# batra-mlp-lab/visdial

Measured on AMD Instinct MI355X. Metric: QA-rounds/sec training mn-att-ques-im-hist+disc (batch 20x10x100), higher is better.
Workload: dtype f32 operands and results; the option recurrence multiplies the EXACT 3-way bf16 split of both operands (9 bf16 MFMA products per fp32 product, f32 accumulate: fp32-grade, errors at the f32 MFMA's own level) -- its two step kernels and its weight-gradient contraction; f32 MFMA (v_mfma_f32_32x32x2_f32

## Files before the change

visdial_amd/csrc/common.h:

```cpp
#pragma once
#include <hip/hip_runtime.h>
#include <stdint.h>
#include <stdio.h>
#include <string.h>

#define VD_OK 0
#define VD_ERR_ARG -1
#define VD_ERR_HIP -2
#define VD_ERR_STATE -3
#define VD_FLAG_BF16 1
#define VD_FLAG_SPLIT9 2
#define VD_FLAG_SPLIT6 4
#define VD_FLAG_SPLIT3 8
#define VD_FLAG_SPLIT (VD_FLAG_SPLIT9 | VD_FLAG_SPLIT6 | VD_FLAG_SPLIT3)
#define VD_FLAG_LIVE_PREFIX 16
#define VD_FLAG_STATE_ONLY 32
#define VD_FLAG_TREE 64
#define VD_FLAG_HOLD 128
#define VD_LIVE_PREFIX_ROWS 128
#define VD_BEAM_LMAX 64

void vd_set_error(const char* fmt, ...);

#define VD_CHECK_ARG(cond, ...)                                   \
// ... 32 lines not shown
  float* wht = nullptr;
  size_t wht_bytes = 0;
  unsigned* sync = nullptr;
  size_t sync_bytes = 0;
};
int vd_stream_scratch(hipStream_t stream, size_t wht_bytes, size_t sync_bytes, VdStreamScratch* out);
int vd_num_cus();

struct VdZeroSet {
  float* buf[6];
  int ncols[6];
  int n;
  long quads_per_row;
};
int vd_zero_inactive_multi(const VdZeroSet& z, const int32_t* nact_dev, int T, int N, hipStream_t stream);

typedef unsigned short vd_bf16_bits;
int vd_lstm_forward_c16(const vd_bf16_bits* table16, int64_t tab_ld, const int32_t* tok_gather, const float* Wh, vd_bf16_bits* gates16,
                        vd_bf16_bits* h16, float* h_last, float* c, int T, int N, int H, hipStream_t stream);
int vd_lstm_backward_c16(const float* Wh, vd_bf16_bits* gates16, const float* c, const float* dh_last, float* dc_work, int T, int N, int H,
                         hipStream_t stream);
int vd_f32_to_bf16(const float* src, vd_bf16_bits* dst, int64_t n, hipStream_t stream);
int vd_gemm_tn_acc_bf16(const vd_bf16_bits* A16, const vd_bf16_bits* B16, float* C, int64_t ldc, int M, int N, int K, hipStream_t stream);
int vd_segment_rowsum_acc_bf16(const vd_bf16_bits* X16, int64_t ldx, const int32_t* tok, const int32_t* perm, int64_t n, int ncol,
                               float* out, int64_t ldo, hipStream_t stream);

int vd_bf16_shadow_get(int slot, const float* base, size_t floats, vd_bf16_bits** out);
const vd_bf16_bits* vd_bf16_shadow_find(const float* p, size_t floats);
void vd_bf16_shadow_invalidate(const float* p, size_t floats);

// ... 70 lines not shown
```

visdial_amd/csrc/gemm_core.h:

```cpp
#pragma once
#include <stdint.h>
#include <stdlib.h>
#include <type_traits>

#include "common.h"

#ifdef VD_TIMING
#define VD_TSLOTS 12
#define VD_TBLOCKS 8192
static __device__ unsigned long long vd_tbuf[VD_TBLOCKS * VD_TSLOTS];
#define VD_TSTAMP(i, clk)                                                                \
  do {                                                                                   \
    if (threadIdx.x == 0 && blockIdx.x < VD_TBLOCKS) vd_tbuf[blockIdx.x * VD_TSLOTS + (i)] = (clk); \
  } while (0)
#define VD_T(i) VD_TSTAMP(i, __builtin_amdgcn_s_memtime())
#define VD_TREAL(i) VD_TSTAMP(i, __builtin_amdgcn_s_memrealtime())
#else
#define VD_T(i) do {} while (0)
#define VD_TREAL(i) do {} while (0)
#endif

template <int WM_, int WK_, int NT_, int KW_, int DB_ = 1, int MINW_ = 1, int LDSMIN_ = 0, int BF16_ = 0>
struct GemmCfg {
  static constexpr int WM = WM_, WK = WK_, NT = NT_, KW = KW_, DB = DB_, MINW = MINW_;
// ... 713 lines not shown
    attr_set = true;
  }
  const int rotate = rotate_in >= 0 ? rotate_in : 1;
  int grid = tiles_m * tiles_n * splits;
  if constexpr (EpiDeadOf<Epi>::value) {
    VD_CHECK_ARG(splits == 1, "launch_gemm_glds: an epilogue with a row-tile predicate takes no split-K");
    grid = (tiles_m + 7) / 8 * 8 * tiles_n;
  }
  const int lds = Cfg::LDS_BYTES;
  hipLaunchKernelGGL(kern, dim3(grid), dim3(Cfg::THREADS), lds, stream, M, N, K,
                     kchunk, tiles_m, tiles_n, rotate, A, lda, B, ldb, e);
  VD_LAUNCH_CHECK();
  return VD_OK;
}

template <class Prob, int MAXP>
struct GroupArgs {
  Prob p[MAXP];
  int tile_start[MAXP + 1];
  int nprob;
};

template <class Cfg, class Prob, int MAXP>
__global__ void __launch_bounds__(Cfg::THREADS, Cfg::MINW)
gemm_f32_grouped_kernel(GroupArgs<Prob, MAXP> g) {
  extern __shared__ __attribute__((aligned(16))) float smem[];
  if constexpr (Cfg::WK > 1) __builtin_amdgcn_s_setprio(3);
  const int wg = xcd_remap(blockIdx.x, gridDim.x);
  int pi = 0;
#pragma unroll
// ... 68 lines not shown
  __device__ __forceinline__ void operator()(const f32x16 (&acc)[NT], int row0, int col0, int lane, int M,
                                             int N, float*  = nullptr) const {
#pragma unroll
    for (int j = 0; j < NT; ++j) {
      const int col = col0 + j * 32 + (lane & 31);
      if (col >= N) continue;
#pragma unroll
      for (int r = 0; r < 16; ++r) {
        const int row = row0 + mfma_row(r, lane);
        if (row >= M) continue;
        unsafeAtomicAdd(C + (long)row * ldc + col, acc[j][r]);
      }
    }
  }
};

template <class Cfg, class ASrc, class BSrc, class Epi>
static int launch_gemm(int M, int N, int K, int splits, ASrc a, BSrc b, Epi e, hipStream_t stream) {
  if (M <= 0 || N <= 0) return VD_OK;
  const int tiles_m = vd_cdiv(M, Cfg::BM), tiles_n = vd_cdiv(N, Cfg::BN);
  if (splits < 1) splits = 1;
  int kchunk = K > 0 ? vd_cdiv(vd_cdiv(K, splits), Cfg::BK) * Cfg::BK : Cfg::BK;
  if (K > 0) splits = vd_cdiv(K, kchunk);
  else splits = 1;
  auto kern = gemm_f32_kernel<Cfg, ASrc, BSrc, Epi>;
  static bool attr_set = false;
  if (!attr_set) {
    VD_HIP(hipFuncSetAttribute(reinterpret_cast<const void*>(kern), hipFuncAttributeMaxDynamicSharedMemorySize,
                               Cfg::LDS_BYTES));
    attr_set = true;
// ... 13 lines not shown
```

visdial_amd/csrc/gemm_ops.hip:

```cpp
#include "gemm_core.h"
#include "split_core.h"

using CfgBigDB = GemmCfg<4, 1, 4, 32>;
using CfgBig = GemmCfg<4, 1, 4, 16, 0, 3>;
using CfgSmall = GemmCfg<1, 4, 1, 32, 0, 3>;

static inline bool use_small(int M, int N) {
  return (long)vd_cdiv(M, CfgBig::BM) * vd_cdiv(N, CfgBig::BN) < 48;
}

static int check_align(const void* p, long ld, const char* what) {
  if (((uintptr_t)p & 15) != 0 || (ld & 3) != 0) {
    vd_set_error("%s: pointer must be 16-byte aligned and leading dimension a multiple of 4 (ld=%ld)", what, ld);
    return VD_ERR_ARG;
  }
  return VD_OK;
}

__global__ void colsum_kernel(const float* __restrict__ X, long ld, int M, int N, int rows_per_block,
                              float* __restrict__ out) {
  const int col = blockIdx.x * blockDim.x + threadIdx.x;
  if (col >= N) return;
  const int r0 = blockIdx.y * rows_per_block;
  const int r1 = min(M, r0 + rows_per_block);
// ... 461 lines not shown
    return VD_OK;
  }
  const int cb = vd_cdiv(N, 256);
  int rb = vd_cdiv(1024, cb);
  int rows_per_block = vd_cdiv(M, rb);
  if (rows_per_block < 16) rows_per_block = 16;
  rb = vd_cdiv(M, rows_per_block);
  hipLaunchKernelGGL(colsum_kernel, dim3(cb, rb), dim3(256), 0, (hipStream_t)stream, X, ld, M, N,
                     rows_per_block, out);
  VD_LAUNCH_CHECK();
  return VD_OK;
}

}

__global__ void __launch_bounds__(256) bf16_tn_tail_kernel(const vd_bf16_bits* __restrict__ A, const vd_bf16_bits* __restrict__ B, float* __restrict__ C,
                                                           long ldc, int M, int N, int K) {
  const long i = (long)blockIdx.x * 256 + threadIdx.x;
  if (i >= (long)M * N) return;
  const int m = (int)(i / N), n = (int)(i % N);
  float acc = 0.f;
  for (int k = 0; k < K; ++k)
    acc += __uint_as_float((unsigned)A[(long)k * M + m] << 16) * __uint_as_float((unsigned)B[(long)k * N + n] << 16);
  unsafeAtomicAdd(C + (long)m * ldc + n, acc);
}
int vd_gemm_tn_acc_bf16(const vd_bf16_bits* A16, const vd_bf16_bits* B16, float* C, int64_t ldc, int M, int N, int K, hipStream_t stream) {
  VD_CHECK_ARG(A16 && B16 && C && M % 128 == 0 && N % 128 == 0 && K >= 0, "vd_gemm_tn_acc_bf16: M, N must be multiples of 128");
  const int K1 = K & ~31;
  if (K1 > 0) {
    const bool big = M % 256 == 0 && N % 256 == 0 && K1 >= 8192;
// ... 10 lines not shown
```

visdial_amd/csrc/paths.h:

```cpp
#pragma once
#include "common.h"

static inline int vd_precision_flags(int lstmBf16) {
  switch (lstmBf16) {
    case 0: return 0;
    case 1: return VD_FLAG_BF16;
    case 3: return VD_FLAG_SPLIT3;
    case 6: return VD_FLAG_SPLIT6;
    case 9: return VD_FLAG_SPLIT9;
    default: return -1;
  }
}
static inline int vd_split_nprod(int flags) {
  return (flags & VD_FLAG_SPLIT9) ? 9 : (flags & VD_FLAG_SPLIT6) ? 6 : (flags & VD_FLAG_SPLIT3) ? 3 : 0;
}

constexpr long VD_THROUGHPUT_ROWS = 2048;
constexpr int VD_LSTM_FWD_TILE_BIG = 128, VD_LSTM_FWD_TILE_SMALL = 32;
static inline int vd_lstm_fwd_row_tile(long N) { return N >= VD_THROUGHPUT_ROWS ? VD_LSTM_FWD_TILE_BIG : VD_LSTM_FWD_TILE_SMALL; }
static inline bool vd_lstm_glds_fwd_fits(long N, int H) { return N >= VD_THROUGHPUT_ROWS && H % 32 == 0 && N * H * 4 < (1L << 32); }
static inline bool vd_lstm_glds_bwd_fits(long N, int H) { return N >= VD_THROUGHPUT_ROWS && H % 32 == 0 && N * 4 * H * 4 < (1L << 32); }
static inline bool vd_lstm_bf16_fits(long N, int H) { return N >= VD_THROUGHPUT_ROWS && H % 32 == 0; }
static inline bool vd_lstm_c16_fits(long N, int H) { return N >= VD_THROUGHPUT_ROWS && H % 128 == 0; }

static inline bool vd_tn_kmajor_fits(long M, long N, long K) { return M % 128 == 0 && N % 128 == 0 && K >= 1024; }
constexpr int VD_SPLIT_TN_BM = 256, VD_SPLIT_TN_BN = 128;
static inline bool vd_tn_split_tiles(long M, long N) { return M % VD_SPLIT_TN_BM == 0 && N % VD_SPLIT_TN_BN == 0; }

static inline bool vd_img_split_ok(long rows, int H, int Kc) {
  return rows >= 128 && H % 16 == 0 && Kc % 16 == 0 && rows * (H > Kc ? H : Kc) * 4 < (1L << 32);
}

static inline bool vd_lhood_fused_fits(long rows, long ldh, long V, long ldw, int H) {
  return H >= 64 && H % 16 == 0 && V >= 128 && ldh % 4 == 0 && ldw % 4 == 0 && rows * ldh * 4 < (1L << 32) && V * ldw * 4 < (1L << 32);
}
static inline bool vd_lhood_prefix_fits(int T, long rows) { return T >= 1 && T < 256 && rows >= 1; }
```

visdial_amd/csrc/rt_core.h:

```cpp
#pragma once
#include <math.h>
#include <stdarg.h>
#include <stdlib.h>
#include <string.h>

#include <algorithm>
#include <map>
#include <memory>
#include <numeric>
#include <random>
#include <string>
#include <vector>

#include "../../include/visdial_hip.h"
#include "common.h"
#include "paths.h"
#include "rt_switches.h"

static_assert(VD_OK == 0 && VD_ERR_ARG == -1, "rt_switches.h returns the two as literals: it includes no common.h");

int vd_lstm2_forward_p(const vd_lstm2_fwd_t* st, int nstacks, int H, int flags, hipStream_t stream);
int vd_lstm2_backward_p(const vd_lstm2_bwd_t* st, int nstacks, int H, int flags, hipStream_t stream);

int vd_img_drop_gather(const float* pre, const uint8_t* mask1, float* xdrop, int N, int R, int S2, int H, float scale, hipStream_t stream);
int vd_img_common_forward_p(const float* pre, const uint8_t* mask1, const float* xdrop, const float* Wc, const float* bc, const float* qc,
                            const uint8_t* mask2, float* iqc, int N, int R, int S2, int H, int Kc, float scale, int flags, hipStream_t stream);
int vd_img_tr_backward_p(const float* dz, const float* Wc, const float* p, const float* datt, const uint8_t* mask1, float* dpre, int N, int R,
                         int S2, int H, int Kc, float scale, int flags, hipStream_t stream);
int vd_img_common_wgrad_p(const float* dz, const float* pre, const uint8_t* mask1, const float* xdrop, float* dWc, int N, int R, int S2, int H,
                          int Kc, float scale, int flags, hipStream_t stream);

int vd_mn_attention_round_p(const float* Q, int64_t q_ld, const float* Hm, float* P, float* hAtt, float* Qout, int B, int R, int r, int H,
// ... 59 lines not shown
};

struct DevBuf {
  void* p = nullptr;
  size_t bytes = 0;
};

struct SeqTok {
  int T = 0, N = 0;
  bool present = false, sorted = false;
  int32_t* tok = nullptr;
  std::vector<int32_t> nact;
  int32_t *tok_sorted = nullptr, *fwd_idx = nullptr, *inv_idx = nullptr, *perm = nullptr, *inv = nullptr, *nact_dev = nullptr;
  int32_t *act = nullptr, *act1 = nullptr, *prev1 = nullptr;
  int n_act = 0, n_act1 = 0;
};

struct TreeChunk {
  int o0 = 0, C = 0, Tl = 0, Nw = 0;
  long n_nodes = 0;
  std::vector<int32_t> widths;
  int32_t* mask2 = nullptr;
  int32_t* node_row = nullptr;
  int32_t *enode = nullptr, *etgt = nullptr;
};

struct BatchSlot {
  int B = 0;
  bool tree_ok = false;
  std::vector<TreeChunk> tree;
  SeqTok q, h, opt, ain, aout, oin, oout;
  float* img = nullptr;
  int32_t* gt = nullptr;
  std::vector<int32_t> gt_host;
  bool has_gt = false;
  int32_t* opt_uid = nullptr;
  int opt_total = 0;
  int32_t *opt_sort_off = nullptr, *opt_sort_perm = nullptr;
  bool cached = false;
  uint64_t cache_stamp = 0;
  std::vector<int32_t> miss_keys, opt_host;
  hipEvent_t ready = nullptr;
  hipEvent_t done = nullptr;
  bool used = false;
  bool uploaded = false;
  std::map<std::string, DevBuf> bufs, pinned;
};

struct RowIndex {
  int T = 0;
  std::vector<int32_t> keys;
  std::vector<int32_t> table;
  int32_t size() const { return T ? (int32_t)(keys.size() / (size_t)T) : 0; }
  void reset(int T_) {
    T = T_;
    keys.clear();
// ... 28 lines not shown
  }
};

struct OptionCache {
  long capacity = 0;
  RowIndex index;
  float* table = nullptr;
  long table_rows = 0;
  uint64_t stamp = 1;
  void flush() {
    index.reset(index.T);
    ++stamp;
  }
};
static constexpr long VD_OPTION_CACHE_FIRST_ROWS = 16384;

struct Encoder;
struct Decoder;

}

struct vd_model {
  vd_model_params p;
  int flags = 0;
  std::string enc_name, dec_name;
  std::vector<vdrt::Tensor> spec;
  std::map<std::string, int> index;
  long numel = 0;
  float *W = nullptr, *G = nullptr, *M = nullptr, *V = nullptr;
  std::map<std::string, vdrt::DevBuf> ws;
  std::map<std::string, vdrt::DevBuf> ext_masks;
  hipStream_t s_main = nullptr, s_side = nullptr;
  hipStream_t s_wg = nullptr;
  bool wg_active = false, wg_used = false;
  std::vector<hipEvent_t> ev_pool;
  size_t ev_next = 0;
  hipEvent_t ev_enc_grads = nullptr;
  hipEvent_t ev_updated = nullptr;
  bool updated_recorded = false;
  bool enc_grads_recorded = false;
  hipEvent_t ev_loss = nullptr, ev_prof[6] = {nullptr, nullptr, nullptr, nullptr, nullptr, nullptr};
  bool training = true, streams = true, prof_valid = false;
  long step = 0;
  int adam_t = 0;
  double lr = 1e-3;
  vdrt::BatchSlot slot[2];
  int cur = -1, uploaded = -1;
  float* loss_host = nullptr;
  long loss_cap = 0, loss_n = 0;
// ... 68 lines not shown
  VD_HIP(hipEventRecord(e, from));
  VD_HIP(hipStreamWaitEvent(side, e, 0));
  return VD_OK;
}
inline int join_stream(vd_model* m, hipStream_t side, hipStream_t to) { return fork_stream(m, side, to); }
inline hipStream_t side_stream(vd_model* m, hipStream_t cur) { return m->streams ? m->s_side : cur; }
inline int wg_fork(vd_model* m, hipStream_t cur, hipStream_t* out) {
  *out = cur;
  if (!m->wg_active || !m->s_wg) return VD_OK;
  VD_TRY(fork_stream(m, cur, m->s_wg));
  m->wg_used = true;
  *out = m->s_wg;
  return VD_OK;
}

inline int drop_mask(vd_model* m, const std::string& site, size_t numel, float p, hipStream_t s, uint8_t** out) {
  *out = nullptr;
  if (!m->training || p <= 0.f) return VD_OK;
  auto it = m->ext_masks.find(site);
  if (it != m->ext_masks.end()) {
    VD_CHECK_ARG(it->second.bytes >= numel, "dropout mask '%s' holds %zu bytes, the batch needs %zu", site.c_str(),
                 it->second.bytes, numel);
    *out = static_cast<uint8_t*>(it->second.p);
    return VD_OK;
  }
  if (!m->ext_masks.empty()) {
    vd_set_error("external dropout masks are set but none for site '%s'", site.c_str());
    return VD_ERR_STATE;
  }
  uint8_t* buf = nullptr;
// ... 200 lines not shown
      } else {
        VD_TRY(vd_gemm_nn(x, D, Wx(m), 4 * H, Wp(m, name + ".b"), gates, 4 * H, T * N, (int)(4 * H), (int)D, 0, s));
      }
      VD_TRY(vd_lstm_forward(gates, (int64_t)N * 4 * H, 4 * H, nullptr, mask, Wh(m), h0, c0, gates_out, h, c, T, N, (int)H, flags, s));
    }
    if (h_out) *h_out = h;
    return VD_OK;
  }
  int param_grads(vd_model* m, hipStream_t s, const std::vector<bool>& need_dx, std::vector<float*>* dxs) {
    const long TN = (long)T * N;
    float* dW = Gp(m, name + ".W");
    float* dWh = dW + D * 4 * H;
    const bool by_rows = rows && rows->act;
    auto dense_fits = [&](long Mrows, long K) { return vd_tn_kmajor_fits(Mrows, 4 * H, K); };
    auto wg_flags = [&](long Mrows) { return (m->flags & VD_FLAG_BF16) && vd_tn_split_tiles(Mrows, 4 * H) ? VD_FLAG_BF16 : 0; };
    if (by_rows && !(T > 1 && dense_fits(H, (long)(T - 1) * N))) {
      if (rows->n_act1 > 0)
        VD_TRY(vd_gemm_tn_rows_acc(h, H, rows->prev1, gates, 4 * H, rows->act1, dWh, 4 * H, (int)H, (int)(4 * H), rows->n_act1, s));
    } else if (T > 1) {
      VD_TRY(vd_gemm_tn_acc(h, H, gates + (long)N * 4 * H, 4 * H, dWh, 4 * H, (int)H, (int)(4 * H), (T - 1) * N, wg_flags(H), s));
    }
    if (h0) VD_TRY(vd_gemm_tn_acc(h0, H, gates, 4 * H, dWh, 4 * H, (int)H, (int)(4 * H), N, 0, s));
    VD_TRY(vd_colsum_acc(gates, 4 * H, (int)TN, (int)(4 * H), Gp(m, name + ".b"), s));
    if (dxs) dxs->assign(parts.size(), nullptr);
    long roff = 0;
    for (size_t i = 0; i < parts.size(); ++i) {
      if (by_rows && !dense_fits(parts[i], TN)) {
        if (rows->n_act > 0)
          VD_TRY(vd_gemm_tn_rows_acc(xs[i], parts[i], rows->act, gates, 4 * H, rows->act, dW + roff * 4 * H, 4 * H, (int)parts[i],
                                     (int)(4 * H), rows->n_act, s));
      } else {
        VD_TRY(vd_gemm_tn_acc(xs[i], parts[i], gates, 4 * H, dW + roff * 4 * H, 4 * H, (int)parts[i], (int)(4 * H), (int)TN, wg_flags(parts[i]), s));
      }
      if (need_dx.empty() || need_dx[i]) {
        float* dx;
        VD_TRY(ws_get(m, name + ".dx" + std::to_string(i), (size_t)TN * parts[i], &dx));
        VD_TRY(vd_gemm_nt(gates, 4 * H, Wx(m) + roff * 4 * H, 4 * H, nullptr, dx, parts[i], (int)TN, (int)parts[i], (int)(4 * H),
                          VD_ACT_NONE, 0, s));
        if (dxs) (*dxs)[i] = dx;
      }
      roff += parts[i];
    }
// ... 47 lines not shown
```

visdial_amd/csrc/rt_decoders.h:

```cpp
#pragma once
#include "rt_encoders.h"

namespace vdrt {

int option_cache_resolve(vd_model* m, BatchSlot& sl, const int32_t* options, long NO, int To, hipStream_t s);

struct Decoder {
  virtual ~Decoder() {}
  virtual void declare(vd_model* m) = 0;
  virtual int forward_backward(vd_model* m, BatchSlot& b, bool only_forward) = 0;
  virtual int retrieve(vd_model* m, BatchSlot& b) = 0;
  virtual int retrieve_lhood(vd_model*, BatchSlot&) {
    vd_set_error("vd_model_retrieve_lhood: the live-row log-likelihood head scores candidates of decoder 'gen'; this model's decoder is 'disc'");
    return VD_ERR_ARG;
  }
  virtual int gen_begin(vd_model*, const int32_t*, int) { return no_gen(); }
  virtual int gen_step(vd_model*, const int32_t*, float*) { return no_gen(); }
  virtual int gen_select(vd_model*, const int32_t*, int) { return no_gen(); }
  virtual int gen_beam_search(vd_model*, int, int, int, int, int32_t*, double*) { return no_gen(); }
  virtual int gen_sample(vd_model*, int, int, int, double, const double*, int32_t*, double*) { return no_gen(); }
  static int no_gen() {
    vd_set_error("sampling / beam search only for the generative decoder (model.lua:436-438)");
    return VD_ERR_STATE;
  }
// ... 136 lines not shown
    m->scores = scores;
    m->prof_valid = !only_forward;
    if (only_forward) return VD_OK;
    VD_TRY(fork_stream(m, s, sd));
    float *dc, *dtab;
    int32_t* perm = b.opt_sort_perm;
    VD_TRY(ws_get(m, "opt.dc", (size_t)NO * H, &dc));
    VD_TRY(ws_get(m, "opt.dtable", (size_t)(V + 1) * 4 * H, &dtab));
    VD_CHECK_ARG(perm, "decoder 'disc': the batch slot carries no option-token sort");
    VD_TRY(vd_memset(dtab, 0, (V + 1) * 4 * H * 4, sd));
    VD_HIP(hipEventRecord(m->ev_prof[2], s));
    m->wg_active = m->streams && m->s_wg && (flags & VD_FLAG_BF16) != 0;
    m->wg_used = false;
    auto enc_bwd = [&]() -> int {
      VdRange r("encoder backward");
      VD_TRY(m->enc->backward(m, sd, b, d_enc));
      VD_PROBE_REC(1, sd);
      if (m->wg_used) VD_PROBE_REC(2, m->s_wg);
      if (m->wg_used) {
        VD_TRY(fork_stream(m, sd, m->s_wg));
        VD_HIP(hipEventRecord(m->ev_enc_grads, m->s_wg));
      } else {
        VD_HIP(hipEventRecord(m->ev_enc_grads, sd));
      }
      m->enc_grads_recorded = true;
      return VD_OK;
    };
    {
      VdRange r("disc: option LSTM backward");
      if (c16) VD_TRY(vd_lstm_backward_c16(Wopt + E * 4 * H, gates16, c, d_optH, dc, To, NO, (int)H, s));
      else VD_TRY(vd_lstm_backward(Wopt + E * 4 * H, gates, c, nullptr, nullptr, d_optH, nullptr, dc, nullptr, nullptr, nullptr, To, NO, (int)H, flags, s));
    }
    VD_HIP(hipEventRecord(m->ev_prof[3], s));
    VD_TRY(enc_bwd());
    VdRange rwg("disc: table gradient + dWh");
    VD_TRY(fork_stream(m, s, sd));
    if (c16) VD_TRY(vd_segment_rowsum_acc_bf16(gates16, 4 * H, b.opt.tok, perm, (long)To * NO, (int)(4 * H), dtab, 4 * H, sd));
    else VD_TRY(vd_segment_rowsum_acc(gates, 4 * H, b.opt.tok, perm, (long)To * NO, (int)(4 * H), dtab, 4 * H, sd));
    VD_TRY(vd_colsum_acc(dtab, 4 * H, (int)V + 1, (int)(4 * H), Gp(m, "opt.b"), sd));
    VD_TRY(vd_gemm_tn_acc(Wp(m, "embed"), E, dtab, 4 * H, Gp(m, "opt.W"), 4 * H, (int)E, (int)(4 * H), (int)V + 1, 0, sd));
    VD_HIP(hipEventRecord(m->ev_prof[4], s));
    if (To > 1 && c16)
      VD_TRY(vd_gemm_tn_acc_bf16(h16, gates16 + (long)NO * 4 * H, Gp(m, "opt.W") + E * 4 * H, 4 * H, (int)H, (int)(4 * H), (To - 1) * NO, s));
    else if (To > 1)
      VD_TRY(vd_gemm_tn_acc(h, H, gates + (long)NO * 4 * H, 4 * H, Gp(m, "opt.W") + E * 4 * H, 4 * H, (int)H, (int)(4 * H), (To - 1) * NO,
                            flags & (VD_FLAG_BF16 | VD_FLAG_SPLIT9), s));
    VD_HIP(hipEventRecord(m->ev_prof[5], s));
    VD_TRY(vd_gemm_nt(dtab, 4 * H, Wopt, 4 * H, nullptr, Gp(m, "embed"), E, (int)V + 1, (int)E, (int)(4 * H), VD_ACT_NONE, 2, sd));
    VD_PROBE_REC(3, sd);
    VD_TRY(join_stream(m, sd, s));
    if (m->wg_used) VD_TRY(join_stream(m, m->s_wg, s));
// ... 708 lines not shown
```

visdial_amd/csrc/rt_encoders.h:

```cpp
#pragma once
#include "rt_core.h"

namespace vdrt {

struct Encoder {
  virtual ~Encoder() {}
  virtual void declare(vd_model* m) = 0;
  virtual int forward(vd_model* m, hipStream_t s, BatchSlot& b, float** out) = 0;
  virtual int backward(vd_model* m, hipStream_t s, BatchSlot& b, const float* grad_out) = 0;
  virtual int forward_round(vd_model* m, hipStream_t s, BatchSlot& b, int r, float** out) {
    vd_set_error("encoder '%s' has no history: a rollout never asks it for a round pass", m->enc_name.c_str());
    return VD_ERR_STATE;
  }
  float* out_ = nullptr;
  int round_ready(vd_model* m, const BatchSlot& b, bool state = true) const {
    const int N = b.q.N, R = m->p.maxQuesCount;
    VD_CHECK_ARG(out_ && state && N == N / R * R && b.h.N == N, "round pass without a full encoder pass on this batch");
    return VD_OK;
  }
  virtual std::vector<SeqLSTM>* rnnLayers() { return nullptr; }
  virtual int seqLen(const BatchSlot& b) const { return b.q.T; }
};

inline int tick_flags(const vd_model* m) { return m->flags & VD_FLAG_BF16; }
// ... 121 lines not shown
    WaveStack* st[2] = {&hist, &ques};
    const SeqTok* ss[2] = {&b.h, &b.q};
    float* last[2];
    VD_TRY(wave_forward(m, s, st, ss, 2, last));
    *h3 = last[0];
    *q3 = last[1];
    return VD_OK;
  }
  int backward(vd_model* m, hipStream_t s, BatchSlot& b, const float* dq3, const float* dh3) {
    WaveStack* st[2] = {&hist, &ques};
    const SeqTok* ss[2] = {&b.h, &b.q};
    const float* dlast[2] = {dh3, dq3};
    VD_TRY(wave_backward(m, s, st, ss, 2, dlast));
    hipStream_t sw;
    VD_TRY(wg_fork(m, s, &sw));
    for (int k = 0; k < 2; ++k) VD_TRY(st[k]->param_tail(m, sw, *ss[k]));
    return VD_OK;
  }
};

inline int rows_copy(float* dst, long dst_ld, const float* src, long src_ld, long rows, int cols, hipStream_t s) {
  const int64_t ld = src_ld;
  return vd_rows_cat_p(dst, dst_ld, &src, &ld, &cols, 1, rows, s);
}
inline int round_linear(vd_model* m, hipStream_t s, const std::string& name, const float* x, long ldx, long in, long out, int rows, bool tanh,
                        float* y, long ldy) {
  return vd_gemm_nt(x, ldx, Wp(m, name + ".W"), in, Wp(m, name + ".b"), y, ldy, rows, (int)out, (int)in, tanh ? VD_ACT_TANH : VD_ACT_NONE, 0, s);
}
inline int history_round_concat(vd_model* m, hipStream_t s, BatchSlot& b, const std::vector<const SeqLSTM*>& layers, int r, float* cache,
                                const float** last) {
  const int N = b.h.N, W = b.h.T, R = m->p.maxQuesCount, B = N / R, L = (int)layers.size();
  VD_CHECK_ARG(b.h.present && b.q.present && N == B * R && r >= 1 && r < R, "round pass %d of %d rounds over %d history rows", r, R, N);
// ... 105 lines not shown
    }
    const int N = b.h.N, Th = b.h.T;
    const long E = hist[0].D;
    float *hx, *ht;
    VD_TRY(ws_get(m, "h.x", (size_t)Th * N * E, &hx));
    VD_TRY(vd_embed_gather(Wp(m, "embed"), b.h.tok, nullptr, hx, (long)Th * N, (int)E, 1.f, s));
    VD_TRY(lstm_stack_forward(m, s, hist, {hx}, Th, N, b.h.tok, &ht));
    *last = hist.back().out_at(Th - 1);
    return VD_OK;
  }
  int backward(vd_model* m, hipStream_t s, BatchSlot& b, const float* dlast) {
    if (waved(b)) {
      WaveStack* st = &wave;
      const SeqTok* ss = &b.h;
      VD_TRY(wave_backward(m, s, &st, &ss, 1, &dlast));
      return wave.param_tail(m, s, b.h);
    }
    std::vector<float*> dx;
    VD_TRY(lstm_stack_backward(m, s, hist, dlast, nullptr, &dx));
    return vd_embed_scatter_acc(Gp(m, "embed"), b.h.tok, nullptr, dx[0], (long)b.h.T * b.h.N, (int)hist[0].D, 1.f, s);
  }
  int round(vd_model* m, hipStream_t s, BatchSlot& b, int r, float* cache, const float** hl) {
    std::vector<const SeqLSTM*> layers;
    for (const SeqLSTM& l : hist) layers.push_back(&l);
    return history_round(m, s, b, layers, r, cache, hl);
  }
};

inline int image_repeat(vd_model* m, hipStream_t s, const BatchSlot& b, int N, float** out) {
  const int R = m->p.maxQuesCount, F = m->p.imgFeatureSize;
  int32_t* rep;
// ... 581 lines not shown
```

visdial_amd/csrc/runtime.hip:

```cpp
#include "rt_decoders.h"

using namespace vdrt;

vd_model::~vd_model() {}

namespace {

int upload_tokens(BatchSlot& sl, SeqTok& ss, const std::string& tag, const int32_t* rows_major, int N, int T, bool sorted, hipStream_t s,
                  int rollout_R = 0) {
  ss.T = T;
  ss.N = N;
  ss.present = true;
  ss.sorted = sorted;
  const size_t TN = (size_t)T * N;
  const size_t total = sorted ? 7 * TN + 2 * (size_t)N + T : TN;
  int32_t* stage = nullptr;
  VD_TRY(pin_get(sl.pinned, tag + ".stage", total * sizeof(int32_t), (void**)&stage));
  int32_t* tok = stage;
  std::vector<int> len(sorted ? N : 0);
  for (int n = 0; n < N; ++n) {
    int first = T;
    for (int t = 0; t < T; ++t) {
      const int32_t v = rows_major[(size_t)n * T + t];
      tok[(size_t)t * N + n] = v;
      if (v != 0 && first == T) first = t;
    }
    if (sorted) len[n] = rollout_R > 0 && n % rollout_R != 0 ? T : T - first;
  }
  if (sorted) {
    int32_t* tok_sorted = stage + TN;
// ... 18 lines not shown
      for (int i = 0; i < N; ++i) {
        tok_sorted[(size_t)t * N + i] = tok[(size_t)t * N + perm[i]];
        fwd_idx[(size_t)t * N + i] = t * N + perm[i];
        inv_idx[(size_t)t * N + i] = t * N + inv[i];
      }
    }
    int32_t* act = nact + T;
    int na = 0;
    for (int t = 0; t < T; ++t)
      for (int i = 0; i < ss.nact[t]; ++i) act[na++] = t * N + i;
    const int n0 = T > 0 ? ss.nact[0] : 0;
    int32_t* prev1 = act + TN;
    for (int k = n0; k < na; ++k) prev1[k - n0] = act[k] - N;
    ss.n_act = na;
    ss.n_act1 = na - n0;
  }
  int32_t* dev = nullptr;
  VD_TRY(dev_get(sl.bufs, tag + ".dev", total * sizeof(int32_t), (void**)&dev));
  VD_HIP(hipMemcpyAsync(dev, stage, total * sizeof(int32_t), hipMemcpyHostToDevice, s));
  ss.tok = dev;
  if (sorted) {
    ss.tok_sorted = dev + TN;
    ss.fwd_idx = dev + 2 * TN;
    ss.inv_idx = dev + 3 * TN;
    ss.perm = dev + 4 * TN;
    ss.inv = ss.perm + N;
    ss.nact_dev = ss.inv + N;
    ss.act = ss.nact_dev + T;
    ss.act1 = ss.act + (T > 0 ? ss.nact[0] : 0);
    ss.prev1 = ss.act + TN;
  }
  return VD_OK;
}

bool has(const std::string& s, const char* sub) { return s.find(sub) != std::string::npos; }

}

int vdrt::option_cache_resolve(vd_model* m, BatchSlot& sl, const int32_t* options, long NO, int To, hipStream_t s) {
  OptionCache& oc = m->ocache;
  if (oc.index.T != To) {
    oc.index.reset(To);
    ++oc.stamp;
  }
  const int32_t count = oc.index.size();
// ... 689 lines not shown
```

Measured before the change: 8778.

## Group encoder LSTM weight-gradient GEMMs into one stream-K live-row launch

Encoder weight-gradient products (dW and dWh per LSTM layer) are now collected while the encoder backward runs instead of being launched one by one. They are issued together as a single grouped f32 MFMA kernel. The kernel walks only the live, length-sorted rows as k-segments and splits the total k-step work evenly across a fixed number of chunks, stream-K style, accumulating with atomics. This aims to cut per-GEMM launch overhead and load imbalance from ragged sequence lengths. It adds a host-side work plan (cached per batch signature), extra upload bytes, and atomic-accumulation contention. Flushing is deferred to the side stream after the encoder backward.

After: 8900 (median of 6 runs). 1.01x the previous value.

```diff
diff --git a/visdial_amd/csrc/common.h b/visdial_amd/csrc/common.h
--- a/visdial_amd/csrc/common.h
+++ b/visdial_amd/csrc/common.h
@@ -70,6 +70,17 @@
   long quads_per_row;
 };
 int vd_zero_inactive_multi(const VdZeroSet& z, const int32_t* nact_dev, int T, int N, hipStream_t stream);
+
+constexpr int VD_LIVE_MAXP = 8;
+struct VdLiveProduct {
+  const float *A, *B;
+  float* C;
+  const int32_t* segs;
+  long lda, ldb, ldc;
+  int M, N;
+};
+int vd_gemm_tn_live_grouped(const VdLiveProduct* prod, int nprod, const int32_t* items, const int32_t* chunk_start, int chunks,
+                            hipStream_t stream);
 
 typedef unsigned short vd_bf16_bits;
 int vd_lstm_forward_c16(const vd_bf16_bits* table16, int64_t tab_ld, const int32_t* tok_gather, const float* Wh, vd_bf16_bits* gates16,
diff --git a/visdial_amd/csrc/gemm_core.h b/visdial_amd/csrc/gemm_core.h
--- a/visdial_amd/csrc/gemm_core.h
+++ b/visdial_amd/csrc/gemm_core.h
@@ -751,6 +751,166 @@
   return VD_OK;
 }
 
+struct LiveProduct {
+  const float* A;
+  const float* B;
+  float* C;
+  const int4* segs;
+  int lda, ldb, ldc, tiles_n;
+};
+template <int MAXP>
+struct LiveGroupArgs {
+  LiveProduct p[MAXP];
+  const int4* items;
+  const int* chunk_start;
+};
+
+typedef int vd_i32x4 __attribute__((ext_vector_type(4)));
+typedef const vd_i32x4 __attribute__((address_space(4))) vd_const_i32x4;
+__device__ __forceinline__ const vd_const_i32x4* vd_as_const(const void* p) { return (const vd_const_i32x4*)(uintptr_t)p; }
+
+template <class Cfg, class Epi>
+__device__ __forceinline__ void gemm_block_glds_live(int row_base, int col_base, const float* A, long lda, const float* B, long ldb,
+                                                     const int4* __restrict__ segs, int seg, int j, int nk, const Epi& epi, float* smem) {
+  constexpr int WM = Cfg::WM, NT = Cfg::NT, BM = Cfg::BM, BN = Cfg::BN;
+  constexpr int NIA = (BM / 16) / WM, NIB = (BN / 16) / WM;
+  constexpr int ABUF = BM * 16, BBUF = BN * 16;
+  static_assert(Cfg::WK == 1 && Cfg::KW == 16 && BM == 128 && BN == 128 && Cfg::BF16 == 0, "k-major fp32 tiles of 16 x 128");
+  static_assert((3 * ABUF + 2 * BBUF) * 4 <= Cfg::LDS_BYTES && (3 * ABUF + 3 * BBUF) * 4 > Cfg::LDS_BYTES,
+                "three A buffers and two B buffers: the ring below is written for that request distance");
+  const int tid = (int)threadIdx.x, lane = tid & 63;
+  const int wm = __builtin_amdgcn_readfirstlane(tid >> 6);
+  const int hi = lane >> 5, l31 = lane & 31;
+
+  f32x16 acc[NT];
+#pragma unroll
+  for (int jj = 0; jj < NT; ++jj)
+#pragma unroll
+    for (int r = 0; r < 16; ++r) acc[jj][r] = 0.f;
+
+  const vd_const_i32x4* const ctab = vd_as_const(segs);
+  vd_i32x4 sg = ctab[seg];
+  auto next = [&]() {
+    const int d = ((sg.x + j * 16) << 5) | (j + 1 == sg.y ? sg.z : 16);
+    if (++j == sg.y) {
+      sg = ctab[++seg];
+      j = 0;
+    }
+    return d;
+  };
+
+  unsigned voffa[NIA], voffb[NIB];
+#pragma unroll
+  for (int i = 0; i < NIA; ++i) voffa[i] = (unsigned)((((long)(i * WM + wm) * 2 + hi) * lda + row_base + l31 * 4) * 4);
+#pragma unroll
+  for (int i = 0; i < NIB; ++i) voffb[i] = (unsigned)((((long)(i * WM + wm) * 2 + hi) * ldb + col_base + l31 * 4) * 4);
+  float* const sA = smem;
+  float* const sB = smem + 3 * ABUF;
+  const unsigned ldsA = (unsigned)(uintptr_t)sA, ldsB = (unsigned)(uintptr_t)sB;
+  auto back = [&](int i, int cnt, long ld) { return (unsigned)(max((i * WM + wm) * 2 + hi - (cnt - 1), 0) * ld * 4); };
+  auto issue_a = [&](int d, int buf) {
+    const float* ak = A + (long)(d >> 5) * lda;
+    const int cnt = d & 31;
+    if (cnt == 16) {
+#pragma unroll
+      for (int i = 0; i < NIA; ++i) glds16(voffa[i], ak, ldsA + buf * (ABUF * 4) + (i * WM + wm) * 1024);
+    } else {
+#pragma unroll
+      for (int i = 0; i < NIA; ++i) glds16(voffa[i] - back(i, cnt, lda), ak, ldsA + buf * (ABUF * 4) + (i * WM + wm) * 1024);
+    }
+  };
+  auto issue_b = [&](int d, int buf) {
+    const float* bk = B + (long)(d >> 5) * ldb;
+    const int cnt = d & 31;
+    if (cnt == 16) {
+#pragma unroll
+      for (int i = 0; i < NIB; ++i) glds16(voffb[i], bk, ldsB + buf * (BBUF * 4) + (i * WM + wm) * 1024);
+    } else {
+#pragma unroll
+      for (int i = 0; i < NIB; ++i) glds16(voffb[i] - back(i, cnt, ldb), bk, ldsB + buf * (BBUF * 4) + (i * WM + wm) * 1024);
+    }
+  };
+  struct Frag {
+    float a[4];
+    float b[NT][4];
+  };
+  auto read_frags = [&](int bufa, int bufb, int half, int d, Frag& f) {
+    const float* sa = sA + bufa * ABUF + (half * 8 + hi) * BM + wm * 32 + l31;
+    const float* sb = sB + bufb * BBUF + (half * 8 + hi) * BN + l31;
+#pragma unroll
+    for (int s4 = 0; s4 < 4; ++s4) {
+      f.a[s4] = sa[s4 * 2 * BM];
+#pragma unroll
+      for (int jj = 0; jj < NT; ++jj) f.b[jj][s4] = sb[s4 * 2 * BN + jj * 32];
+    }
+    const int cnt = d & 31;
+    if (cnt < 16) {
+#pragma unroll
+      for (int s4 = 0; s4 < 4; ++s4)
+        if (half * 8 + hi + s4 * 2 >= cnt) f.a[s4] = 0.f;
+    }
+  };
+  auto mfma16 = [&](const Frag& f) {
+#pragma unroll
+    for (int s4 = 0; s4 < 4; ++s4)
+#pragma unroll
+      for (int jj = 0; jj < NT; ++jj) acc[jj] = __builtin_amdgcn_mfma_f32_32x32x2f32(f.a[s4], f.b[jj][s4], acc[jj], 0, 0, 0);
+  };
+  auto wait_vm = [&](int n) {
+    switch (n) {
+      case 0: asm volatile("s_waitcnt vmcnt(0)" ::: "memory"); break;
+      case 1: asm volatile("s_waitcnt vmcnt(1)" ::: "memory"); break;
+      case 2: asm volatile("s_waitcnt vmcnt(2)" ::: "memory"); break;
+      case 3: asm volatile("s_waitcnt vmcnt(3)" ::: "memory"); break;
+      case 4: asm volatile("s_waitcnt vmcnt(4)" ::: "memory"); break;
+      case 5: asm volatile("s_waitcnt vmcnt(5)" ::: "memory"); break;
+      case 6: asm volatile("s_waitcnt vmcnt(6)" ::: "memory"); break;
+      default: asm volatile("s_waitcnt vmcnt(0)" ::: "memory"); break;
+    }
+  };
+
+  if (nk > 0) {
+    Frag f0, f1;
+    int d0 = next(), d1 = next(), d2 = next();
+    issue_b(d0, 0);
+    issue_a(d0, 0);
+    if (1 < nk) {
+      issue_b(d1, 1);
+      issue_a(d1, 1);
+    }
+    if (2 < nk) issue_a(d2, 2);
+    wait_vm(NIA * (min(nk, 3) - 1) + NIB * (min(nk, 2) - 1));
+    asm volatile("s_barrier" ::: "memory");
+    read_frags(0, 0, 0, d0, f0);
+    int ca = 0, cb = 0;
+    for (int kt = 0; kt < nk; ++kt) {
+      const int na = (ca + 1 == 3) ? 0 : ca + 1, nb = cb ^ 1;
+      read_frags(ca, cb, 1, d0, f1);
+      mfma16(f0);
+      __builtin_amdgcn_sched_barrier(0);
+      if (kt + 3 <= nk) {
+        static_assert(NIA == 2, "steady-state vmcnt immediate");
+        asm volatile("s_waitcnt vmcnt(2)" ::: "memory");
+      } else {
+        wait_vm(NIA * max(0, min(kt + 2, nk - 1) - (kt + 1)) + NIB * max(0, min(kt + 1, nk - 1) - (kt + 1)));
+      }
+      asm volatile("s_waitcnt lgkmcnt(0)\n\ts_barrier" ::: "memory");
+      __builtin_amdgcn_sched_barrier(0);
+      const int d3 = next();
+      if (kt + 2 < nk) issue_b(d2, cb);
+      if (kt + 3 < nk) issue_a(d3, ca);
+      if (kt + 1 < nk) read_frags(na, nb, 0, d1, f0);
+      mfma16(f1);
+      ca = na;
+      cb = nb;
+      d0 = d1;
+      d1 = d2;
+      d2 = d3;
+    }
+  }
+  epi(acc, row_base + wm * 32, col_base, lane, 1 << 30, 1 << 30, smem + wm * 1024);
+}
+
 template <class Prob, int MAXP>
 struct GroupArgs {
   Prob p[MAXP];
@@ -849,6 +1009,36 @@
     }
   }
 };
+
+template <class Cfg, int MAXP>
+__global__ void __launch_bounds__(Cfg::THREADS, Cfg::MINW)
+gemm_f32_live_grouped_kernel(LiveGroupArgs<MAXP> g) {
+  extern __shared__ __attribute__((aligned(16))) float smem[];
+  const int wg = xcd_remap(blockIdx.x, gridDim.x);
+  const int i0 = g.chunk_start[wg], i1 = g.chunk_start[wg + 1];
+  for (int it = i0; it < i1; ++it) {
+    const vd_i32x4 item = vd_as_const(g.items)[it];
+    const LiveProduct& P = g.p[item.x >> 24];
+    const int tile = item.x & 0xffffff;
+    const EpiAtomic<Cfg::NT> e{P.C, (long)P.ldc};
+    gemm_block_glds_live<Cfg>((tile / P.tiles_n) * Cfg::BM, (tile % P.tiles_n) * Cfg::BN, P.A, P.lda, P.B, P.ldb, P.segs, item.y, item.z,
+                              item.w, e, smem);
+  }
+}
+
+template <class Cfg, int MAXP>
+static int launch_live_grouped(const LiveGroupArgs<MAXP>& g, int chunks, hipStream_t stream) {
+  if (chunks <= 0) return VD_OK;
+  auto kern = gemm_f32_live_grouped_kernel<Cfg, MAXP>;
+  static bool attr_set = false;
+  if (!attr_set) {
+    VD_HIP(hipFuncSetAttribute(reinterpret_cast<const void*>(kern), hipFuncAttributeMaxDynamicSharedMemorySize, Cfg::LDS_BYTES));
+    attr_set = true;
+  }
+  hipLaunchKernelGGL(kern, dim3(chunks), dim3(Cfg::THREADS), Cfg::LDS_BYTES, stream, g);
+  VD_LAUNCH_CHECK();
+  return VD_OK;
+}
 
 template <class Cfg, class ASrc, class BSrc, class Epi>
 static int launch_gemm(int M, int N, int K, int splits, ASrc a, BSrc b, Epi e, hipStream_t stream) {
diff --git a/visdial_amd/csrc/gemm_ops.hip b/visdial_amd/csrc/gemm_ops.hip
--- a/visdial_amd/csrc/gemm_ops.hip
+++ b/visdial_amd/csrc/gemm_ops.hip
@@ -499,6 +499,26 @@
 
 }
 
+int vd_gemm_tn_live_grouped(const VdLiveProduct* prod, int nprod, const int32_t* items, const int32_t* chunk_start, int chunks,
+                            hipStream_t stream) {
+  using Cfg = GemmCfg<4, 1, 4, 16, 0, 4, 41984>;
+  VD_CHECK_ARG(prod && nprod >= 1 && nprod <= VD_LIVE_MAXP && items && chunk_start && chunks >= 0, "vd_gemm_tn_live_grouped: bad args");
+  LiveGroupArgs<VD_LIVE_MAXP> g{};
+  for (int i = 0; i < nprod; ++i) {
+    const VdLiveProduct& p = prod[i];
+    VD_CHECK_ARG(p.A && p.B && p.C && p.segs && p.M > 0 && p.N > 0 && p.M % Cfg::BM == 0 && p.N % Cfg::BN == 0 && p.lda >= p.M && p.ldb >= p.N &&
+                     16 * p.lda * 4 < (1L << 31) && 16 * p.ldb * 4 < (1L << 31) && p.ldc < (1L << 31) &&
+                     (long)(p.M / Cfg::BM) * (p.N / Cfg::BN) < (1 << 24),
+                 "vd_gemm_tn_live_grouped: product %d: M=%d N=%d", i, p.M, p.N);
+    if (int rc = check_align(p.A, p.lda, "vd_gemm_tn_live_grouped A")) return rc;
+    if (int rc = check_align(p.B, p.ldb, "vd_gemm_tn_live_grouped B")) return rc;
+    g.p[i] = LiveProduct{p.A, p.B, p.C, reinterpret_cast<const int4*>(p.segs), (int)p.lda, (int)p.ldb, (int)p.ldc, p.N / Cfg::BN};
+  }
+  g.items = reinterpret_cast<const int4*>(items);
+  g.chunk_start = chunk_start;
+  return launch_live_grouped<Cfg, VD_LIVE_MAXP>(g, chunks, stream);
+}
+
 __global__ void __launch_bounds__(256) bf16_tn_tail_kernel(const vd_bf16_bits* __restrict__ A, const vd_bf16_bits* __restrict__ B, float* __restrict__ C,
                                                            long ldc, int M, int N, int K) {
   const long i = (long)blockIdx.x * 256 + threadIdx.x;
diff --git a/visdial_amd/csrc/paths.h b/visdial_amd/csrc/paths.h
--- a/visdial_amd/csrc/paths.h
+++ b/visdial_amd/csrc/paths.h
@@ -27,6 +27,10 @@
 constexpr int VD_SPLIT_TN_BM = 256, VD_SPLIT_TN_BN = 128;
 static inline bool vd_tn_split_tiles(long M, long N) { return M % VD_SPLIT_TN_BM == 0 && N % VD_SPLIT_TN_BN == 0; }
 
+static inline bool vd_wgrad_group_fits(bool sorted_rows, long M, long N, int flags) {
+  return sorted_rows && M % 128 == 0 && N % 128 == 0 && !(flags & VD_FLAG_BF16);
+}
+
 static inline bool vd_img_split_ok(long rows, int H, int Kc) {
   return rows >= 128 && H % 16 == 0 && Kc % 16 == 0 && rows * (H > Kc ? H : Kc) * 4 < (1L << 32);
 }
diff --git a/visdial_amd/csrc/rt_core.h b/visdial_amd/csrc/rt_core.h
--- a/visdial_amd/csrc/rt_core.h
+++ b/visdial_amd/csrc/rt_core.h
@@ -16,6 +16,7 @@
 #include "common.h"
 #include "paths.h"
 #include "rt_switches.h"
+#include "wgrad_plan.h"
 
 static_assert(VD_OK == 0 && VD_ERR_ARG == -1, "rt_switches.h returns the two as literals: it includes no common.h");
 
@@ -105,6 +106,9 @@
   int32_t *tok_sorted = nullptr, *fwd_idx = nullptr, *inv_idx = nullptr, *perm = nullptr, *inv = nullptr, *nact_dev = nullptr;
   int32_t *act = nullptr, *act1 = nullptr, *prev1 = nullptr;
   int n_act = 0, n_act1 = 0;
+  std::vector<vdplan::Seg> seg_host[2];
+  int32_t* seg_dev[2] = {nullptr, nullptr};
+  int seg_ksteps[2] = {0, 0};
 };
 
 struct TreeChunk {
@@ -131,6 +135,9 @@
   bool cached = false;
   uint64_t cache_stamp = 0;
   std::vector<int32_t> miss_keys, opt_host;
+  std::vector<long> wgrad_sig;
+  int32_t *wgrad_items = nullptr, *wgrad_chunk_start = nullptr;
+  int wgrad_chunks = 0;
   hipEvent_t ready = nullptr;
   hipEvent_t done = nullptr;
   bool used = false;
@@ -189,6 +196,12 @@
   }
 };
 static constexpr long VD_OPTION_CACHE_FIRST_ROWS = 16384;
+
+struct WgradProduct {
+  VdLiveProduct p;
+  const SeqTok* rows;
+  int t_first;
+};
 
 struct Encoder;
 struct Decoder;
@@ -208,6 +221,8 @@
   hipStream_t s_main = nullptr, s_side = nullptr;
   hipStream_t s_wg = nullptr;
   bool wg_active = false, wg_used = false;
+  std::vector<vdrt::WgradProduct> wgrad;
+  bool wgrad_open = false, wgrad_hold = false;
   std::vector<hipEvent_t> ev_pool;
   size_t ev_next = 0;
   hipEvent_t ev_enc_grads = nullptr;
@@ -306,6 +321,59 @@
   return VD_OK;
 }
 
+constexpr int VD_WGRAD_CHUNKS = 768, VD_WGRAD_MIN_KSTEPS = 32;
+inline void wgrad_begin(vd_model* m) {
+  m->wgrad.clear();
+  m->wgrad_open = true;
+}
+inline int wgrad_flush(vd_model* m, BatchSlot& b, hipStream_t s) {
+  m->wgrad_open = false;
+  const int n = (int)m->wgrad.size();
+  if (n == 0) return VD_OK;
+  VD_CHECK_ARG(n <= VD_LIVE_MAXP, "%d weight-gradient products in one encoder backward, the grouped launch takes %d", n, VD_LIVE_MAXP);
+  VdLiveProduct lp[VD_LIVE_MAXP];
+  vdplan::Product prod[VD_LIVE_MAXP];
+  std::vector<long> sig;
+  long total = 0;
+  for (int i = 0; i < n; ++i) {
+    const WgradProduct& w = m->wgrad[i];
+    const int f = w.t_first;
+    lp[i] = w.p;
+    lp[i].segs = w.rows->seg_dev[f];
+    prod[i] = vdplan::Product{w.rows->seg_host[f].data(), (int)w.rows->seg_host[f].size() - 1, w.rows->seg_ksteps[f], (w.p.M / 128) * (w.p.N / 128)};
+    total += (long)prod[i].ksteps * prod[i].tiles;
+    for (const long v : {(long)(intptr_t)w.rows, (long)f, (long)w.p.M, (long)w.p.N}) sig.push_back(v);
+  }
+  m->wgrad.clear();
+  if (total == 0) return VD_OK;
+  if (sig != b.wgrad_sig) {
+    std::vector<vdplan::Item> items;
+    std::vector<int32_t> start;
+    const int chunks = (int)std::min<long>(VD_WGRAD_CHUNKS, (total + VD_WGRAD_MIN_KSTEPS - 1) / VD_WGRAD_MIN_KSTEPS);
+    vdplan::work_list(prod, n, chunks, &items, &start);
+    const size_t ints = 4 * items.size() + start.size();
+    int32_t *stage, *dev;
+    VD_TRY(pin_get(b.pinned, "wgrad.plan", ints * sizeof(int32_t), (void**)&stage));
+    VD_TRY(dev_get(b.bufs, "wgrad.plan", ints * sizeof(int32_t), (void**)&dev));
+    for (size_t i = 0; i < items.size(); ++i) {
+      const vdplan::Item& it = items[i];
+      const int32_t packed[4] = {(it.product << 24) | it.tile, it.seg, it.j, it.nk};
+      memcpy(stage + 4 * i, packed, sizeof(packed));
+    }
+    memcpy(stage + 4 * items.size(), start.data(), start.size() * sizeof(int32_t));
+    VD_HIP(hipMemcpyAsync(dev, stage, ints * sizeof(int32_t), hipMemcpyHostToDevice, s));
+    b.wgrad_items = dev;
+    b.wgrad_chunk_start = dev + 4 * items.size();
+    b.wgrad_chunks = chunks;
+    b.wgrad_sig = sig;
+  }
+  return vd_gemm_tn_live_grouped(lp, n, b.wgrad_items, b.wgrad_chunk_start, b.wgrad_chunks, s);
+}
+inline int wgrad_end(vd_model* m, BatchSlot& b, hipStream_t s) {
+  m->wgrad_open = false;
+  return m->wgrad_hold ? VD_OK : wgrad_flush(m, b, s);
+}
+
 inline int drop_mask(vd_model* m, const std::string& site, size_t numel, float p, hipStream_t s, uint8_t** out) {
   *out = nullptr;
   if (!m->training || p <= 0.f) return VD_OK;
@@ -536,7 +604,13 @@
     const bool by_rows = rows && rows->act;
     auto dense_fits = [&](long Mrows, long K) { return vd_tn_kmajor_fits(Mrows, 4 * H, K); };
     auto wg_flags = [&](long Mrows) { return (m->flags & VD_FLAG_BF16) && vd_tn_split_tiles(Mrows, 4 * H) ? VD_FLAG_BF16 : 0; };
-    if (by_rows && !(T > 1 && dense_fits(H, (long)(T - 1) * N))) {
+    auto grouped = [&](const float* A, long Mrows, const float* B, float* C, int t_first) {
+      if (!m->wgrad_open || !vd_wgrad_group_fits(by_rows, Mrows, 4 * H, m->flags)) return false;
+      m->wgrad.push_back(WgradProduct{VdLiveProduct{A, B, C, nullptr, Mrows, 4 * H, 4 * H, (int)Mrows, (int)(4 * H)}, rows, t_first});
+      return true;
+    };
+    if (T > 1 && grouped(h, H, gates + (long)N * 4 * H, dWh, 1)) {
+    } else if (by_rows && !(T > 1 && dense_fits(H, (long)(T - 1) * N))) {
       if (rows->n_act1 > 0)
         VD_TRY(vd_gemm_tn_rows_acc(h, H, rows->prev1, gates, 4 * H, rows->act1, dWh, 4 * H, (int)H, (int)(4 * H), rows->n_act1, s));
     } else if (T > 1) {
@@ -547,7 +621,8 @@
     if (dxs) dxs->assign(parts.size(), nullptr);
     long roff = 0;
     for (size_t i = 0; i < parts.size(); ++i) {
-      if (by_rows && !dense_fits(parts[i], TN)) {
+      if (grouped(xs[i], parts[i], gates, dW + roff * 4 * H, 0)) {
+      } else if (by_rows && !dense_fits(parts[i], TN)) {
         if (rows->n_act > 0)
           VD_TRY(vd_gemm_tn_rows_acc(xs[i], parts[i], rows->act, gates, 4 * H, rows->act, dW + roff * 4 * H, 4 * H, (int)parts[i],
                                      (int)(4 * H), rows->n_act, s));
diff --git a/visdial_amd/csrc/rt_decoders.h b/visdial_amd/csrc/rt_decoders.h
--- a/visdial_amd/csrc/rt_decoders.h
+++ b/visdial_amd/csrc/rt_decoders.h
@@ -174,7 +174,10 @@
     m->wg_used = false;
     auto enc_bwd = [&]() -> int {
       VdRange r("encoder backward");
-      VD_TRY(m->enc->backward(m, sd, b, d_enc));
+      m->wgrad_hold = true;
+      const int rc = m->enc->backward(m, sd, b, d_enc);
+      m->wgrad_hold = false;
+      VD_TRY(rc);
       VD_PROBE_REC(1, sd);
       if (m->wg_used) VD_PROBE_REC(2, m->s_wg);
       if (m->wg_used) {
@@ -195,6 +198,10 @@
     VD_TRY(enc_bwd());
     VdRange rwg("disc: table gradient + dWh");
     VD_TRY(fork_stream(m, s, sd));
+    if (!m->wgrad.empty()) {
+      VD_TRY(wgrad_flush(m, b, sd));
+      VD_HIP(hipEventRecord(m->ev_enc_grads, sd));
+    }
     if (c16) VD_TRY(vd_segment_rowsum_acc_bf16(gates16, 4 * H, b.opt.tok, perm, (long)To * NO, (int)(4 * H), dtab, 4 * H, sd));
     else VD_TRY(vd_segment_rowsum_acc(gates, 4 * H, b.opt.tok, perm, (long)To * NO, (int)(4 * H), dtab, 4 * H, sd));
     VD_TRY(vd_colsum_acc(dtab, 4 * H, (int)V + 1, (int)(4 * H), Gp(m, "opt.b"), sd));
diff --git a/visdial_amd/csrc/rt_encoders.h b/visdial_amd/csrc/rt_encoders.h
--- a/visdial_amd/csrc/rt_encoders.h
+++ b/visdial_amd/csrc/rt_encoders.h
@@ -159,8 +159,9 @@
     VD_TRY(wave_backward(m, s, st, ss, 2, dlast));
     hipStream_t sw;
     VD_TRY(wg_fork(m, s, &sw));
+    wgrad_begin(m);
     for (int k = 0; k < 2; ++k) VD_TRY(st[k]->param_tail(m, sw, *ss[k]));
-    return VD_OK;
+    return wgrad_end(m, b, sw);
   }
 };
 
@@ -296,7 +297,9 @@
       WaveStack* st = &wave;
       const SeqTok* ss = &b.h;
       VD_TRY(wave_backward(m, s, &st, &ss, 1, &dlast));
-      return wave.param_tail(m, s, b.h);
+      wgrad_begin(m);
+      VD_TRY(wave.param_tail(m, s, b.h));
+      return wgrad_end(m, b, s);
     }
     std::vector<float*> dx;
     VD_TRY(lstm_stack_backward(m, s, hist, dlast, nullptr, &dx));
diff --git a/visdial_amd/csrc/runtime.hip b/visdial_amd/csrc/runtime.hip
--- a/visdial_amd/csrc/runtime.hip
+++ b/visdial_amd/csrc/runtime.hip
@@ -12,8 +12,10 @@
   ss.N = N;
   ss.present = true;
   ss.sorted = sorted;
+  sl.wgrad_sig.clear();
   const size_t TN = (size_t)T * N;
-  const size_t total = sorted ? 7 * TN + 2 * (size_t)N + T : TN;
+  const size_t seg_at = (7 * TN + 2 * (size_t)N + T + 3) / 4 * 4, seg_ints = 4 * ((size_t)T + 1);
+  const size_t total = sorted ? seg_at + 2 * seg_ints : TN;
   int32_t* stage = nullptr;
   VD_TRY(pin_get(sl.pinned, tag + ".stage", total * sizeof(int32_t), (void**)&stage));
   int32_t* tok = stage;
@@ -62,6 +64,10 @@
     for (int k = n0; k < na; ++k) prev1[k - n0] = act[k] - N;
     ss.n_act = na;
     ss.n_act1 = na - n0;
+    for (int f = 0; f < 2; ++f) {
+      ss.seg_ksteps[f] = vdplan::live_segments(ss.nact.data(), T, N, f, &ss.seg_host[f]);
+      memcpy(stage + seg_at + f * seg_ints, ss.seg_host[f].data(), ss.seg_host[f].size() * sizeof(vdplan::Seg));
+    }
   }
   int32_t* dev = nullptr;
   VD_TRY(dev_get(sl.bufs, tag + ".dev", total * sizeof(int32_t), (void**)&dev));
@@ -77,6 +83,7 @@
     ss.act = ss.nact_dev + T;
     ss.act1 = ss.act + (T > 0 ? ss.nact[0] : 0);
     ss.prev1 = ss.act + TN;
+    for (int f = 0; f < 2; ++f) ss.seg_dev[f] = dev + seg_at + f * seg_ints;
   }
   return VD_OK;
 }
diff --git a/visdial_amd/csrc/wgrad_plan.h b/visdial_amd/csrc/wgrad_plan.h
--- /dev/null
+++ b/visdial_amd/csrc/wgrad_plan.h
@@ -0,0 +1,78 @@
+#pragma once
+#include <stdint.h>
+
+#include <vector>
+
+namespace vdplan {
+
+constexpr int KSTEP = 16;
+
+struct Seg {
+  int32_t row;
+  int32_t nks;
+  int32_t tail;
+  int32_t kfirst;
+};
+
+struct Item {
+  int32_t product, tile;
+  int32_t seg, j;
+  int32_t nk;
+};
+
+inline int live_segments(const int32_t* nact, int T, int N, int t_first, std::vector<Seg>* out) {
+  out->clear();
+  int total = 0;
+  for (int t = t_first; t < T; ++t) {
+    const int n = nact[t] < N ? nact[t] : N;
+    if (n <= 0) continue;
+    int full = (n + KSTEP - 1) / KSTEP;
+    if (full > N / KSTEP) full = N / KSTEP;
+    const int rest = n - full * KSTEP;
+    const int nks = full + (rest > 0 ? 1 : 0);
+    out->push_back(Seg{(t - t_first) * N, nks, rest > 0 ? rest : KSTEP, total});
+    total += nks;
+  }
+  out->push_back(Seg{0, 1 << 30, KSTEP, total});
+  return total;
+}
+
+struct Product {
+  const Seg* segs;
+  int nseg;
+  int ksteps;
+  int tiles;
+};
+
+inline void work_list(const Product* prod, int nprod, int chunks, std::vector<Item>* items, std::vector<int32_t>* chunk_start) {
+  items->clear();
+  chunk_start->assign(1, 0);
+  long total = 0;
+  for (int p = 0; p < nprod; ++p) total += (long)prod[p].ksteps * prod[p].tiles;
+  if (chunks < 1) chunks = 1;
+  const long q = total / chunks, r = total % chunks;
+  int p = 0, tile = 0, seg = 0, j = 0, k = 0;
+  auto skip_empty = [&]() { while (p < nprod && (prod[p].ksteps == 0 || prod[p].tiles == 0)) ++p; };
+  skip_empty();
+  for (int w = 0; w < chunks; ++w) {
+    long left = q + (w < r ? 1 : 0);
+    while (left > 0) {
+      const Product& P = prod[p];
+      const int nk = (int)(left < P.ksteps - k ? left : P.ksteps - k);
+      items->push_back(Item{p, tile, seg, j, nk});
+      left -= nk;
+      k += nk;
+      if (k == P.ksteps) {
+        k = seg = j = 0;
+        if (++tile == P.tiles) { tile = 0; ++p; skip_empty(); }
+      } else {
+        int adv = nk;
+        while (adv >= P.segs[seg].nks - j) { adv -= P.segs[seg].nks - j; ++seg; j = 0; }
+        j += adv;
+      }
+    }
+    chunk_start->push_back((int32_t)items->size());
+  }
+}
+
+}
```
